# Cobalt-27/CompactFusion

Measured on AMD Instinct MI355X. Metric: residual_compressed_activation_exchange_throughput, higher is better.
Workload: dtype f16

## Files before the change

compactfusion_amd/csrc/cfx_absmean.hip:

```cpp
#include <hip/hip_runtime.h>
#include <hip/hip_ext.h>
#include <stdint.h>
#include <stdio.h>
#include <stdlib.h>
#include <string.h>
#include <algorithm>
#include "cfx.h"
#include "cfx_internal.h"
#include "cfx_device.h"
#include "cfx_host.h"

#define CFX_I_FLAG_LR_FACTORS_ONLY 0x100
#define CFX_I_FLAG_LR_ABS 0x200
extern "C" CFX_HIDDEN size_t cfx_i_lr_workspace_bytes_any(int N, int C, int rank, int batch);
extern "C" CFX_HIDDEN void cfx_i_lr_factor_offsets(int N, int C, int rank, size_t* offU16, size_t* offV16, size_t* per);

template <bool EMIT_BITS, int US, bool WT = false, int NW = WAVES, bool PUB = false, bool KEEP = false, bool TAG = false, class E = ElemF16>
__device__ __forceinline__ void absmean_stats_body(const cfx_comp_item& it, int N, int C, int R, int CB, int bx, int by,
                                                   u64* rowpart, u64 (*sm)[TILE_C], Probe probe = Probe(),
                                                   h16x8* xk = nullptr, h16x8* bk = nullptr, TagArena ta = TagArena()) {
#define SSTAMP(k) probe.at(k)
    const TileCoord t = tile_coord_at(bx, by, N, C, R);
    const int cb = bx;
    u64* colpart = rowpart + (size_t)N * CB;
    const h16* x = (const h16*)it.x;
    const h16* base = (const h16*)it.base;
    unsigned char* bitsout = (unsigned char*)it.packet;
    const int C8 = C >> 3;

    double col[8];
#pragma unroll
    for (int i = 0; i < 8; ++i) col[i] = 0.0;

    for (int r = t.r0 + t.w; r < t.r1; r += NW * US) {
        h16x8 xv[US], bv[US];
#pragma unroll
        for (int j = 0; j < US; ++j) {
            const int rr = r + NW * j;
            xv[j] = (h16x8)(h16)0;
            bv[j] = (h16x8)(h16)0;
            if (rr < t.r1 && t.act) {
                xv[j] = EMIT_BITS ? ld8nt(x + (size_t)rr * C + t.c) : ld8(x + (size_t)rr * C + t.c);
                if (base) bv[j] = ld8(base + (size_t)rr * C + t.c);
// ... 35 lines not shown
        }
        SSTAMP(9);
        u64 tot = 0;
#pragma unroll
        for (int j = 0; j < US; ++j) {
            const unsigned lo = wave_sum_u32_dpp((unsigned)(rs[j] & 0xffffffu));
            const unsigned hi = wave_sum_u32_dpp((unsigned)(rs[j] >> 24));
            const u64 tj = ((u64)hi << 24) + lo;
            if ((t.lane >> 4) == j) tot = tj;
        }
        SSTAMP(10);
        if ((t.lane & 15) == 0 && (t.lane >> 4) < US) {
            const int rr = r + NW * (t.lane >> 4);
            if (rr < t.r1) {
                if (TAG) put_tagged(ta.trow, rowpart, (size_t)cb * N + rr, tot, ta.tagbits);
                else if (WT) put_part(part32_of(rowpart, N, C, CB), rowpart, (size_t)cb * N + rr, tot);
                else rowpart[(size_t)cb * N + rr] = tot;
            }
        }
    }
#pragma unroll
    for (int i = 0; i < 8; ++i) sm[t.w][i * 64 + (t.lane ^ (i << 3))] = (u64)(col[i] * 16777216.0);
    SSTAMP(11);
    if (TAG && EMIT_BITS) asm volatile("s_waitcnt vmcnt(0)" ::: "memory");
    if (WT) lds_barrier(); else __syncthreads();
    SSTAMP(12);
    for (int k = threadIdx.x; k < TILE_C; k += NW * 64) {
        const int s = (k & 7) * 64 + ((k >> 3) ^ ((k & 7) << 3));
        const int cc = bx * TILE_C + k;
        if (cc < C) {
            u64 v = 0;
#pragma unroll
            for (int w = 0; w < NW; ++w) v += sm[w][s];
            if (TAG) put_tagged(ta.tcol, colpart, (size_t)by * C + cc, v, ta.tagbits);
            else if (WT) put_part(part32_of(rowpart, N, C, CB) + (size_t)N * CB, colpart, (size_t)by * C + cc, v);
            else colpart[(size_t)by * C + cc] = v;
        }
    }
#undef SSTAMP
}

template <bool EMIT_BITS, class E>
__global__ __launch_bounds__(NTHR) void k_absmean_stats(BatchC batch, int N, int C, int R, u64* ws, size_t ws_stride) {
    __shared__ u64 sm[WAVES][TILE_C];
    absmean_stats_body<EMIT_BITS, UNROLL_S, false, WAVES, false, false, false, E>(batch.it[blockIdx.z], N, C, R, gridDim.x, blockIdx.x, blockIdx.y, ws + (size_t)blockIdx.z * ws_stride, sm);
}

template <int NT>
__device__ __forceinline__ void absmean_finalize_body(const cfx_comp_item& it, int N, int C, int CB, int P, int per_byte, int eps_mode,
                                                      const u64* rowpart, int bx, u64* smem) {
    const u64* colpart = rowpart + (size_t)N * CB;
    h16* U = (h16*)((char*)it.packet + (size_t)N * (C / per_byte));
    h16* V = U + N;
    const int tid = threadIdx.x;
    if (bx == 0) {
        constexpr int KEEP = 3;
        u64 srow[KEEP];
        u64 acc = 0;
        int it_n = 0;
        for (int n = tid; n < N; n += NT, ++it_n) {
// ... 416 lines not shown
        for (int n0 = tid + 2 * NT; n0 - tid < N; n0 += 2 * NT) {
            const int n1 = n0 + NT;
            u64 s0, s1;
            row_sums2_wt(rowpart, row32, N, CB, min(n0, N - 1), min(n1, N - 1), (n1 & ~63) < N, s0, s1);
            if (n0 < N) PUT16(&U[n0], (h16)((float)mean16(s0, C) / den));
            if (n1 < N) PUT16(&U[n1], (h16)((float)mean16(s1, C) / den));
        }
        if (tid == 0) st_wt(tick + TICK_ALL, 0u);
    }
    if (last_col) {
        if (c < C) PUT16(&V[c], vmean);
        if (tid == 0) st_wt(tick + 1 + bx, 0u);
    }
#undef PUT16
    if (GATED) {
        asm volatile("s_waitcnt vmcnt(0)" ::: "memory");
        lds_barrier();
        if (tid == 0) gate_arrive_few(gate, (last_all ? 1u : 0u) + (last_col ? 1u : 0u));
    }
    STAMP(6);
#undef STAMP
}

__device__ __forceinline__ void absmean_tagged_jobs(const cfx_comp_item& it, int N, int C, int CB, int P, int bx, u64* rowpart, const TagArena& ta,
                                                    int per_byte, int eps_mode, u64 (*sm)[TILE_C], bool do_col, bool do_row, Probe probe,
                                                    unsigned* gate, unsigned* err, long long timeout) {
    constexpr int NT = FUSED_NT;
#define STAMP(k) probe.at(k)
    lds_barrier();
    const int tid = threadIdx.x;
    const u64* colpart = rowpart + (size_t)N * CB;
    h16* U = (h16*)((char*)it.packet + (size_t)N * (C / per_byte));
    h16* V = U + N;
    SpinClock clk;
    bool failed = false;
#define PUT16(ptr, val) st_wt((u16*)(ptr), hbits(val))
    if (do_col) {
        const int c = bx * TILE_C + tid, cc = min(c, C - 1);
        u64 a = 0;
        for (int p0 = 0; p0 < P && !failed; p0 += FUSED_CH) {
            u64 v[FUSED_CH];
            for (;;) {
#pragma unroll
                for (int j = 0; j < FUSED_CH; ++j) v[j] = ld_wt(&ta.tcol[(size_t)min(p0 + j, P - 1) * C + cc]);
                bool ok = true;
#pragma unroll
                for (int j = 0; j < FUSED_CH; ++j) ok = ok && tag_is(v[j], ta.tagbits);
                if (ok) break;
                __builtin_amdgcn_s_sleep(2);
                if (clk.expired(timeout)) { failed = true; break; }
            }
#pragma unroll
            for (int j = 0; j < FUSED_CH; ++j) {
                const u64 w = v[j] & TAG_SAT;
                if (p0 + j < P) a += (w == TAG_SAT && !failed) ? ld_wt(&colpart[(size_t)(p0 + j) * C + cc]) : w;
            }
        }
        STAMP(4);
        failed = __syncthreads_or(failed ? 1 : 0) != 0;
        if (!failed) {
            if (c < C) {
                const h16 vm = mean16(a, N);
                st_wt(&ta.tV[c], ta.tagbits | (u64)hbits(vm));
                PUT16(&V[c], vm);
            }
            asm volatile("s_waitcnt vmcnt(0)" ::: "memory");
            lds_barrier();
            if (tid == 0) gate_arrive_few(gate, 1u);
        }
        STAMP(5);
    }
    if (do_row && !failed) {
        u64* smem = &sm[1][0];
        auto row_sum = [&](int n) {
            const int nc = min(n, N - 1);
            u64 s_ = 0;
            for (int k0 = 0; k0 < CB && !failed; k0 += FUSED_RCH) {
                u64 q[FUSED_RCH];
                for (;;) {
#pragma unroll
                    for (int j = 0; j < FUSED_RCH; ++j) q[j] = ld_wt(&ta.trow[(size_t)min(k0 + j, CB - 1) * N + nc]);
                    bool ok = true;
#pragma unroll
                    for (int j = 0; j < FUSED_RCH; ++j) ok = ok && tag_is(q[j], ta.tagbits);
                    if (ok) break;
                    __builtin_amdgcn_s_sleep(2);
                    if (clk.expired(timeout)) { failed = true; break; }
                }
#pragma unroll
                for (int j = 0; j < FUSED_RCH; ++j) {
                    const u64 w = q[j] & TAG_SAT;
                    if (k0 + j < CB) s_ += (w == TAG_SAT && !failed) ? ld_wt(&rowpart[(size_t)(k0 + j) * N + nc]) : w;
                }
            }
// ... 77 lines not shown
        const int rr = t.r0 + t.w + NW * j;
        if (t.lane < 8 * US && rr < t.r1 && bx * TILE_C + seg * 64 < C)
            st16_wt(pk + (size_t)rr * (C >> 2) + bx * (TILE_C >> 2) + seg * 16, *(const u32x4*)(smw + j * 128 + seg * 16));
    }
    asm volatile("s_waitcnt vmcnt(0)" ::: "memory");
    lds_barrier();
    if (threadIdx.x == 0) {
        st_wt(&ta.tdone[(size_t)bx * ((N + R - 1) / R) + by], ta.tagbits);
        gate_arrive(gate2, 1u, expect2);
    }
    if (upd) {
#pragma unroll
        for (int j = 0; j < US; ++j) {
            const int rr = t.r0 + t.w + NW * j;
            const h16 tk = hfrom((u16)__builtin_amdgcn_readlane((int)ul, j));
            if (rr < t.r1 && t.act) {
                const h16x8 recv = int2_recv(codes[j], ch8 * tk);
                st8nt(nb + (size_t)rr * C + t.c, ef ? (el_state<E>(has_base, bk[j], recv)) : xk[j]);
            }
        }
    }
}

template <bool EMIT_BITS, int US, bool GATED = false, bool KEEP = false, class E = ElemF16>
__device__ __forceinline__ void absmean_fused_body(const cfx_comp_item& it, int N, int C, int R, int CB, int P, int bx, int by,
                                                   u64* rowpart, unsigned* tick, int per_byte, int eps_mode, u64 (*sm)[TILE_C], int dbg,
                                                   Probe probe, unsigned* gate = nullptr, unsigned gate_expect = 0, int flags = 0,
                                                   unsigned* gate2 = nullptr, unsigned expect2 = 0, unsigned* err = nullptr, long long timeout = 0,
                                                   TagArena ta = TagArena()) {
#define STAMP(k) probe.at(k)
    STAMP(0);
#ifdef CFX_DEV_PROBES
    if (dbg == 3) return;
    if (dbg == 4) {
        const TileCoord t = tile_coord_at(bx, by, N, C, R);
        h16x8 acc = (h16x8)(h16)0;
        for (int r = t.r0 + t.w; r < t.r1; r += FUSED_NW * US) {
            h16x8 xv[US], bv[US];
#pragma unroll
            for (int j = 0; j < US; ++j) {
                const int rr = min(r + FUSED_NW * j, t.r1 - 1);
                xv[j] = ld8nt((const h16*)it.x + (size_t)rr * C + min(t.c, C - 8));
                bv[j] = ld8((const h16*)it.base + (size_t)rr * C + min(t.c, C - 8));
            }
#pragma unroll
            for (int j = 0; j < US; ++j) acc += xv[j] - bv[j];
        }
        if (acc[0] == (h16)12345.0f) ((h16*)it.packet)[threadIdx.x] = acc[1];
        return;
    }
#endif
    h16x8 xk[KEEP ? US : 1], bk[KEEP ? US : 1];
    absmean_stats_body<EMIT_BITS, US, true, FUSED_NW, GATED, KEEP, GATED, E>(it, N, C, R, CB, bx, by, rowpart, sm, probe, xk, bk, ta);
    STAMP(1);
    if constexpr (GATED) {
        const bool v_wg = by == P - 1;
        const bool u_wg = P >= 2 ? (by == P - 2 && bx == CB - 1) : (bx == CB - 1);
        probe.copy(2, 1); probe.copy(3, 1); probe.set(7, (v_wg ? 1 : 0) | (u_wg ? 2 : 0));
        if (v_wg || u_wg) {
            u32x4* park = (u32x4*)&sm[FUSED_NW][0];
            if constexpr (KEEP) {
                park[threadIdx.x] = __builtin_bit_cast(u32x4, xk[US - 1]);
                park[FUSED_NT + threadIdx.x] = __builtin_bit_cast(u32x4, bk[US - 1]);
            }
            absmean_tagged_jobs(it, N, C, CB, P, bx, rowpart, ta, per_byte, eps_mode, sm, v_wg, u_wg, probe, gate, err, timeout);
            if constexpr (KEEP) {
                xk[US - 1] = __builtin_bit_cast(h16x8, park[threadIdx.x]);
                bk[US - 1] = __builtin_bit_cast(h16x8, park[FUSED_NT + threadIdx.x]);
            }
        }
    } else {
    asm volatile("s_waitcnt vmcnt(0)" ::: "memory");
    __syncthreads();
    STAMP(2);
#ifdef CFX_DEV_PROBES
    if (dbg == 1) return;
#endif
    unsigned* flag = (unsigned*)&sm[0][0];
    if (threadIdx.x == 0) flag[0] = __hip_atomic_fetch_add(tick + 1 + bx, 1u, __ATOMIC_RELAXED, __HIP_MEMORY_SCOPE_AGENT);
    if (threadIdx.x == 64) (void)__hip_atomic_fetch_add(tick + TICK_ALL, 1u, __ATOMIC_RELAXED, __HIP_MEMORY_SCOPE_AGENT);
    lds_barrier();
    const bool last_col = flag[0] == (unsigned)(P - 1);
    const bool u_wg = bx == 0 && by == 0;
    STAMP(3);
    probe.set(7, (last_col ? 1 : 0) | (u_wg ? 2 : 0));
#ifdef CFX_DEV_PROBES
    if (dbg == 2) {
        if (last_col && threadIdx.x == 0) st_wt(tick + 1 + bx, 0u);
// ... 30 lines not shown
    int n_st;
    int dq_R, dq_rb;
    int per_byte, eps_mode;
    int dbg;
    u64* ws;
    size_t ws_stride;
    unsigned* tick;
    Probe probe;
    int n_g, g_R, g_rb, n_gt;
    unsigned* gate;
    unsigned gate_expect;
    unsigned* gate_err;
    long long timeout;
    u64* tarena; size_t tarena_stride; unsigned tag;
    signed char src[CFX_MAX_BATCH];
    unsigned* xgate;
    unsigned xexpect;
    int remote;
    P2PInline p2p;
};
#ifndef GATE_WPE
#define GATE_WPE 4
#endif
template <bool EMIT_BITS, int US, bool GATED, bool ST, class E>
__global__ __launch_bounds__(FUSED_NT, GATE_WPE) __attribute__((amdgpu_num_vgpr(52))) void k_absmean_compress(BatchC batch, BatchD ride, BatchD gated, FusedArgs a) {
    __shared__ u64 sm[FUSED_NW][TILE_C];
    int b = blockIdx.x;
    if (b < a.n_st) {
        const int per = a.CB * a.P;
        const int z = b / per, rem = b - z * per;
        const int by = rem / a.CB;
        absmean_fused_body<EMIT_BITS, US, GATED, false, E>(batch.it[z], a.N, a.C, a.R, a.CB, a.P, rem - by * a.CB, by, a.ws + (size_t)z * a.ws_stride,
                                                 a.tick + z * TICK_WORDS, a.per_byte, a.eps_mode, sm, a.dbg,
                                                 a.probe.of(b), a.gate, a.gate_expect, 0, nullptr, 0u, a.gate_err, a.timeout,
                                                 tag_arena_of(a.tarena, a.tarena_stride, z, a.N, a.C, a.CB, a.P, a.tag));
        if constexpr (GATED) {
            if (b == 0 && a.p2p.own) p2p_exchange_inline(a.gate, a.gate_expect, 1, a.p2p, a.xgate, a.xexpect, a.gate_err);
        }
        return;
    }
    if constexpr (EMIT_BITS) {
        b -= a.n_st;
        if constexpr (GATED) {
            if (b < a.n_g) {
                const int per = a.CB * a.g_rb;
                for (int t = b; t < a.n_gt; t += a.n_g) {
                    const int item = t / per, rem = t - item * per;
                    const int ty = rem / a.CB;
                    const int sz = a.src[item];
                    const TagArena ta = tag_arena_of(a.tarena, a.tarena_stride, sz >= 0 ? sz : 0, a.N, a.C, a.CB, a.P, a.tag);
                    binary_dequant_gated_body<FUSED_NW, GATE_KR, 0, ST, E>(gated.it[item], a.N, a.C, a.g_R, rem - ty * a.CB, ty, a.xgate ? a.xgate : a.gate,
                                                                a.xgate ? a.xexpect : a.gate_expect, a.gate_err, a.timeout,
                                                                nullptr,
                                                                a.probe.of(blockIdx.x), a.remote != 0 && sz < 0,
                                                                ONEBIT_D_TAGGED && sz >= 0, ta, (u16*)&sm[0][0]);
                }
                return;
            }
            b -= a.n_g;
        }
        const int per = a.CB * a.dq_rb;
        const int item = b / per, rem = b - item * per;
        const int ty = rem / a.CB;
        binary_dequant_body<FUSED_NW, UNROLL, E>(ride.it[item], a.N, a.C, a.dq_R, rem - ty * a.CB, ty);
    }
}

#ifndef PIPE_US
#define PIPE_US 2
#endif
#define PIPE_MAX_DQ CFX_PIPE_MAX_DQ
struct BatchDX { cfx_decomp_item it[PIPE_MAX_DQ]; };
struct PipeArgs {
    int N, C, CB;
    int n_fin, fin_bpi, fin_P;
    int n_st, st_R, st_P;
    int dq_R, dq_rb;
    const u64* ws_fin;
    u64* ws_st;
    size_t ws_stride;
};
template <bool STEADY>
__global__ __launch_bounds__(NTHR) __attribute__((amdgpu_waves_per_eu(8, 8))) void k_binary_pipe(BatchDX dq, BatchC fin, BatchC st, PipeArgs a) {
    __shared__ u64 sm[WAVES][TILE_C];
    int b = blockIdx.x;
    if (b < a.n_fin) {
        const int item = b / a.fin_bpi;
        absmean_finalize_body<NTHR>(fin.it[item], a.N, a.C, a.CB, a.fin_P, 8, 0, a.ws_fin + (size_t)item * a.ws_stride, b - item * a.fin_bpi, &sm[0][0]);
// ... 198 lines not shown
    }
}

#ifndef INT2_D_TAGGED
#define INT2_D_TAGGED 1
#endif
struct Int2LayerArgs {
    int N, C, CB, R, P, n_st;
    int g_R, g_rb, n_g;
    int flags;
    u64* ws;
    size_t ws_stride;
    unsigned* tick;
    unsigned* gate1; unsigned expect1;
    unsigned* gate2; unsigned expect2;
    unsigned* err;
    long long timeout;
    u64* tarena; size_t tarena_stride; unsigned tag;
    signed char src[CFX_MAX_BATCH];
    unsigned* xgate; unsigned xexpect;
    int remote;
    P2PInline p2p;
};
template <int US, class E>
__global__ __launch_bounds__(FUSED_NT, 4) void k_int2_compress_gated(BatchC batch, BatchD gated, Int2LayerArgs a) {
    __shared__ u64 sm[(GATE_LDS_ROWS > FUSED_NW + 4 ? GATE_LDS_ROWS : FUSED_NW + 4) + 1][TILE_C];
    int b = blockIdx.x;
    if (b < a.n_st) {
        const int per = a.CB * a.P;
        const int z = b / per, rem = b - z * per;
        const int by = rem / a.CB;
        absmean_fused_body<false, US, true, true, E>(batch.it[z], a.N, a.C, a.R, a.CB, a.P, rem - by * a.CB, by, a.ws + (size_t)z * a.ws_stride,
                                                  a.tick + z * TICK_WORDS, 4, 1, sm, 0, Probe(), a.gate1, a.expect1, a.flags, a.gate2, a.expect2, a.err, a.timeout,
                                                  tag_arena_of(a.tarena, a.tarena_stride, z, a.N, a.C, a.CB, a.P, a.tag));
        if (b == 0 && a.p2p.own) p2p_exchange_inline(a.gate2 + 1 * GATE_LINE, a.expect2, 1, a.p2p, a.xgate, a.xexpect, a.err);
        return;
    }
    b -= a.n_st;
    const int per = a.CB * a.g_rb;
    const int item = b / per, rem = b - item * per;
    const int ty = rem / a.CB;
    const int sz = a.src[item];
    const TagArena ta = tag_arena_of(a.tarena, a.tarena_stride, sz >= 0 ? sz : 0, a.N, a.C, a.CB, a.P, a.tag);
    int2_dequant_gated_body<FUSED_NW, GATE_KR2, GATE_KL, E>(gated.it[item], a.N, a.C, a.g_R, rem - ty * a.CB, ty, a.gate2, a.expect2, a.err, a.timeout,
                                                        (u32x4*)&sm[0][0], a.xgate, a.xexpect, a.remote != 0 && sz < 0, INT2_D_TAGGED && sz >= 0, ta, a.R,
                                                        (u16*)&sm[GATE_LDS_ROWS][0]);
}


#define LAUNCH_EL(bf16, ...) do { \
        if (bf16) { using EL = ElemBF16; LAUNCH(__VA_ARGS__); } \
        else { using EL = ElemF16; LAUNCH(__VA_ARGS__); } \
    } while (0)

static bool gated_one_launch(cfx_ctx* ctx, int codec, int C, int CB) {
    return (codec == CFX_CODEC_BINARY || codec == CFX_CODEC_INT2) && ctx->fused && CB <= TICK_MAX_CB && C % 128 == 0 && !ctx->dev_probe && ctx->gated_on;
}

static unsigned abs_arena_for(cfx_ctx* ctx, unsigned ring, void* stream, size_t need_bytes, u64** arena) {
    hipStream_t s = (hipStream_t)stream;
    if (!ctx->mml_arena_owned[ring] || ctx->mml_arena_owner[ring] != stream) {
        if (ctx->mml_arena_owned[ring]) (void)hipDeviceSynchronize();
        ctx->mml_arena_owner[ring] = stream;
        ctx->mml_arena_owned[ring] = true;
    }
    if (ctx->abs_arena_bytes[ring] < need_bytes) {
        if (ctx->abs_arena[ring]) (void)hipFree(ctx->abs_arena[ring]);
        ctx->abs_arena[ring] = nullptr;
        ctx->abs_arena_bytes[ring] = 0;
// ... 90 lines not shown
        ctx->gate_expect[3 * slot + 1] += (unsigned)a.n_st;
        a.expect1 = ctx->gate_expect[3 * slot]; a.expect2 = ctx->gate_expect[3 * slot + 1];
        a.err = ctx->gate_err;
        a.timeout = ctx->gate_timeout;
        a.tarena_stride = tag_arena_words(N, C, CB, P);
        a.tag = abs_arena_for(ctx, slot / TICK_RING, stream, a.tarena_stride * batch * sizeof(u64), &a.tarena);
        if (!a.tag) return fail(ctx, CFX_ERR_LAUNCH, "2-bit layer launch: cannot allocate the partials' arena");
        for (int g_ = 0; g_ < n_gated; ++g_) {
            a.src[g_] = -1;
            for (int i = 0; i < batch; ++i)
                if (gd.it[g_].packet == items[i].packet) a.src[g_] = (signed char)i;
        }
        if (xg) {
            a.xgate = a.gate1 + 2 * GATE_BLOCK;
            a.xexpect = ++ctx->gate_expect[3 * slot + 2];
            a.remote = xg->remote;
            fill_p2p(ctx, xg, a.p2p);
            xg->taken = 1;
            xg->p_gate = a.gate2 + 1 * GATE_LINE;
            xg->p_expect = a.expect2;
            xg->f_gate = a.xgate; xg->f_expect = a.xexpect;
        }
        const dim3 g(a.n_st + a.n_g);
        LAUNCH_EL(bf16, ctx, KID_ABSMEAN_COMPRESS_GATED, s, (k_int2_compress_gated<4, EL>), g, dim3(FUSED_NT), 0, s, b, gd, a);
        return check_launch(ctx, "2-bit layer launch");
    }
    const bool ef_gated = one_launch && codec == CFX_CODEC_BINARY && upd && !(flags & CFX_FLAG_NO_EF) && n_gated + batch <= CFX_MAX_BATCH;
    const bool one_launch_1bit = one_launch && codec == CFX_CODEC_BINARY && (!upd || ef_gated);
    int n_gated_k = n_gated;
    if (ef_gated) {
        for (int i = n_gated - 1; i >= 0; --i) gd.it[i + batch] = gd.it[i];
        for (int i = 0; i < batch; ++i) { gd.it[i].packet = items[i].packet; gd.it[i].base = items[i].base; gd.it[i].recon = items[i].new_base; }
        n_gated_k = n_gated + batch;
    }
    if (fused) {
        FusedArgs a;
        memset(&a, 0, sizeof(a));
        a.N = N; a.C = C; a.CB = CB; a.R = R; a.P = P;
        a.n_st = CB * P * batch;
        a.dq_R = FUSED_NW * UNROLL;
        a.dq_rb = (N + a.dq_R - 1) / a.dq_R;
        a.per_byte = per_byte; a.eps_mode = codec == CFX_CODEC_INT2 ? 1 : 0;
        a.ws = ws; a.ws_stride = wstride; a.tick = tick;
        a.dbg = ctx->dev_probe;
        a.probe = cfx_i_probe(ctx);
        if (one_launch_1bit) {
            a.g_rb = (N + FUSED_NW * GATE_KR - 1) / (FUSED_NW * GATE_KR);
// ... 3 lines not shown
            ctx->gate_expect[3 * slot] += (unsigned)batch * (unsigned)(CB + 1);
            a.gate_expect = ctx->gate_expect[3 * slot];
            a.tarena_stride = tag_arena_words(N, C, CB, P);
            a.tag = abs_arena_for(ctx, slot / TICK_RING, stream, a.tarena_stride * batch * sizeof(u64), &a.tarena);
            if (!a.tag) return fail(ctx, CFX_ERR_LAUNCH, "1-bit layer launch: cannot allocate the partials' arena");
            for (int g_ = 0; g_ < n_gated_k; ++g_) {
                a.src[g_] = -1;
                for (int i = 0; i < batch; ++i)
                    if (gd.it[g_].packet == items[i].packet) a.src[g_] = (signed char)i;
            }
            if (xg) {
                a.xgate = a.gate + GATE_BLOCK;
                a.xexpect = ++ctx->gate_expect[3 * slot + 1];
                a.remote = xg->remote;
                fill_p2p(ctx, xg, a.p2p);
                xg->taken = 1;
                xg->p_gate = a.gate; xg->p_expect = a.gate_expect;
                xg->f_gate = a.xgate; xg->f_expect = a.xexpect;
            }
        }
        a.gate_err = ctx->gate_err;
        a.timeout = ctx->gate_timeout;
        const dim3 g(a.n_st + a.n_g + CB * a.dq_rb * n_ride);
#ifdef CFX_DEV_PROBES
        if (one_launch_1bit && ctx->dev_buf && R % 32 == 0) {
            LAUNCH_EL(bf16, ctx, KID_ABSMEAN_COMPRESS_GATED, s, (k_absmean_compress<true, 4, true, true, EL>), g, dim3(FUSED_NT), 0, s, b, rd, gd, a);
        } else
#endif
        if (one_launch_1bit) {
            LAUNCH_EL(bf16, ctx, KID_ABSMEAN_COMPRESS_GATED, s, (k_absmean_compress<true, 4, true, false, EL>), g, dim3(FUSED_NT), 0, s, b, rd, gd, a);
        } else if (codec == CFX_CODEC_BINARY) {
            if (R % 32 == 0) LAUNCH_EL(bf16, ctx, KID_ABSMEAN_COMPRESS_BITS, s, (k_absmean_compress<true, 4, false, false, EL>), g, dim3(FUSED_NT), 0, s, b, rd, gd, a);
            else LAUNCH_EL(bf16, ctx, KID_ABSMEAN_COMPRESS_BITS, s, (k_absmean_compress<true, 2, false, false, EL>), g, dim3(FUSED_NT), 0, s, b, rd, gd, a);
        } else {
            if (R % 32 == 0) LAUNCH_EL(bf16, ctx, KID_ABSMEAN_COMPRESS, s, (k_absmean_compress<false, 4, false, false, EL>), g, dim3(FUSED_NT), 0, s, b, rd, gd, a);
            else LAUNCH_EL(bf16, ctx, KID_ABSMEAN_COMPRESS, s, (k_absmean_compress<false, 2, false, false, EL>), g, dim3(FUSED_NT), 0, s, b, rd, gd, a);
        }
    } else {
        if (codec == CFX_CODEC_BINARY) LAUNCH_EL(bf16, ctx, KID_ABSMEAN_STATS_BITS, s, (k_absmean_stats<true, EL>), grid, dim3(NTHR), 0, s, b, N, C, R, ws, wstride);
        else LAUNCH_EL(bf16, ctx, KID_ABSMEAN_STATS, s, (k_absmean_stats<false, EL>), grid, dim3(NTHR), 0, s, b, N, C, R, ws, wstride);
        LAUNCH(ctx, KID_ABSMEAN_FINALIZE, s, k_absmean_finalize, dim3(1 + (C + 255) / 256, batch), dim3(1024), 0, s, b, N, C, CB, P, per_byte,
                           codec == CFX_CODEC_INT2 ? 1 : 0, (const u64*)ws, wstride);
        if (n_ride) {
            const int Rr = auto_rows(ctx, N, C, n_ride, false);
            LAUNCH_EL(bf16, ctx, KID_BINARY_DEQUANT, s, (k_binary_dequant<UNROLL, EL>), dim3(CB, (N + Rr - 1) / Rr, n_ride), dim3(NTHR), 0, s, rd, N, C, Rr, (unsigned*)nullptr, 0u);
        }
    }
    if (codec == CFX_CODEC_INT2) {
        LAUNCH_EL(bf16, ctx, KID_INT2_QUANT, s, (k_int2_quant<EL>), gridq, dim3(NTHR), 0, s, b, N, C, Rq, flags);
    } else if (upd && !one_launch_1bit) {
        if (flags & CFX_FLAG_NO_EF) {
            for (int i = 0; i < batch; ++i)
// ... 178 lines not shown
```

compactfusion_amd/csrc/cfx_api.hip:

```cpp
#include <hip/hip_runtime.h>
#include <hip/hip_ext.h>
#include <stdint.h>
#include <stdio.h>
#include <stdlib.h>
#include <string.h>
#include <algorithm>
#include "cfx.h"
#include "cfx_internal.h"
#include "cfx_device.h"
#define CFX_API_TU
#include "cfx_host.h"

__global__ __launch_bounds__(256) void k_residual2_delta(const h16* __restrict__ x, const h16* base, const h16* dbase, h16* dd, size_t n8) {
    const size_t i = (size_t)blockIdx.x * 256 + threadIdx.x;
    if (i >= n8) return;
    const h16x8 d = ld8nt(x + i * 8) - ld8(base + i * 8);
    st8(dd + i * 8, d - ld8(dbase + i * 8));
}
__global__ __launch_bounds__(256) void k_residual2_update(const h16* base, const h16* dbase, const h16* __restrict__ recv, h16* nb, h16* ndb,
                                                          float decay, size_t n8) {
    const size_t i = (size_t)blockIdx.x * 256 + threadIdx.x;
    if (i >= n8) return;
    const h16x8 b = ld8(base + i * 8), d = ld8(dbase + i * 8), r = ld8nt(recv + i * 8);
    const h16x8 pred = b + d;
// ... 142 lines not shown
    c->device = device;
    c->rows_per_tile = 0;
    c->prof = nullptr;
    c->prof_cap = c->prof_n = 0;
    c->prof_stride = 1;
    memset(c->prof_seen, 0, sizeof(c->prof_seen));
    c->prof_mask = 0;
    c->tick = nullptr;
    memset(c->tick_next, 0, sizeof(c->tick_next));
    c->n_ring_streams = 0;
    c->n_cu_cache = 0;
    c->cu_cache_next = 0;
    c->ring_clock = 0;
    memset(c->ring_used, 0, sizeof(c->ring_used));
    c->dev_buf = nullptr;
    c->gate = nullptr;
    c->gate_err = nullptr;
    c->gate_timeout = 500000000LL;
    c->fused = 1;
    c->stats_rows = 0;
    c->gated_on = 1;
    c->lr_chain = c->lr_decode = 0;
    c->dev_probe = 0;
    c->allow_shared_queues = 0;
    c->ipc_kind = 0;
    c->ipc_want = 2;
    c->err[0] = 0;
    return c;
}

int cfx_prepare(cfx_ctx* ctx) {
    if (!ctx) return CFX_ERR_NULL;
    if (ctx->tick) return CFX_OK;
    int cur = -1;
    (void)hipGetDevice(&cur);
    if (cur != ctx->device && hipSetDevice(ctx->device) != hipSuccess) return fail(ctx, CFX_ERR_LAUNCH, "prepare: hipSetDevice failed");
    static_assert(3 * TICK_RING * CFX_RING_STREAMS == sizeof(((cfx_ctx*)0)->gate_expect) / sizeof(unsigned), "gate_expect has three entries per ring slot");
    const size_t tick_words = (size_t)CFX_RING_STREAMS * TICK_RING * CFX_MAX_BATCH * TICK_WORDS;
    const size_t gate_words = (size_t)(CFX_RING_STREAMS * TICK_RING + 1) * GATE_STRIDE;
    const size_t colgate_words = (size_t)CFX_RING_STREAMS * MML_MAX_TILES;
    const size_t bytes = (tick_words + gate_words + colgate_words) * sizeof(unsigned);
    void* p = nullptr;
    int rc = CFX_OK;
    if (hipMalloc(&p, bytes) != hipSuccess || hipMemset(p, 0, bytes) != hipSuccess || hipDeviceSynchronize() != hipSuccess) {
        (void)hipGetLastError();
        if (p) (void)hipFree(p);
// ... 10 lines not shown
    }
    if (cur >= 0 && cur != ctx->device) (void)hipSetDevice(cur);
    return rc;
}

#ifdef CFX_DEV_PROBES
int cfx_dev_stamps(cfx_ctx* ctx, void* buf) {
    if (!ctx) return CFX_ERR_NULL;
    ctx->dev_buf = buf;
    return CFX_OK;
}

int cfx_dev_set_launch_tags(cfx_ctx* ctx, unsigned abs_seq, unsigned mml_seq) {
    if (!ctx) return CFX_ERR_NULL;
    if (!ctx->tick && cfx_prepare(ctx) != CFX_OK) return CFX_ERR_LAUNCH;
    (void)hipDeviceSynchronize();
    ctx->abs_seq = abs_seq;
    ctx->mml_seq = mml_seq;
    return CFX_OK;
}

int cfx_dev_set_probe(cfx_ctx* ctx, int mode) {
    if (!ctx) return CFX_ERR_NULL;
    if (mode < 0 || mode > 4) return fail(ctx, CFX_ERR_BATCH, "dev probe must be 0..4");
    ctx->dev_probe = mode;
    return CFX_OK;
}
#endif

int cfx_set_fused_finalize(cfx_ctx* ctx, int on) {
    if (!ctx) return CFX_ERR_NULL;
    ctx->fused = on != 0;
    return CFX_OK;
}

int cfx_set_stats_rows(cfx_ctx* ctx, int rows) {
    if (!ctx) return CFX_ERR_NULL;
    if (rows < 0 || rows > 4096) return fail(ctx, CFX_ERR_BATCH, "stats rows must be 0 (automatic) .. 4096");
    ctx->stats_rows = rows;
    return CFX_OK;
}

int cfx_set_gated_launch(cfx_ctx* ctx, int on) {
    if (!ctx) return CFX_ERR_NULL;
    ctx->gated_on = on != 0;
    return CFX_OK;
}

int cfx_set_lr_chain(cfx_ctx* ctx, int chain) {
    if (!ctx) return CFX_ERR_NULL;
    if (chain < 0 || chain > 2) return fail(ctx, CFX_ERR_BATCH, "lr chain must be 0 (automatic), 1 (no single launch) or 2 (C-space chain)");
    ctx->lr_chain = chain;
    return CFX_OK;
}

int cfx_set_lr_decode(cfx_ctx* ctx, int mode) {
    if (!ctx) return CFX_ERR_NULL;
    if (mode < 0 || mode > 2) return fail(ctx, CFX_ERR_BATCH, "lr decode must be 0 (automatic), 1 (VALU) or 2 (MFMA)");
    ctx->lr_decode = mode;
    return CFX_OK;
}

int cfx_set_allow_shared_queues(cfx_ctx* ctx, int on) {
    if (!ctx) return CFX_ERR_NULL;
    ctx->allow_shared_queues = on != 0;
    return CFX_OK;
}

// ... 429 lines not shown
```

compactfusion_amd/csrc/cfx_device.h:

```cpp
#ifndef CFX_DEVICE_H
#define CFX_DEVICE_H
#include <hip/hip_runtime.h>
#include <stdint.h>
#include "cfx.h"
#include "cfx_internal.h"

typedef _Float16 h16;
typedef h16 h16x8 __attribute__((ext_vector_type(8)));
typedef unsigned short u16;
typedef u16 u16x8 __attribute__((ext_vector_type(8)));
typedef unsigned long long u64;
typedef unsigned u32x4 __attribute__((ext_vector_type(4)));
typedef float f32x2 __attribute__((ext_vector_type(2)));
typedef h16 h16x2 __attribute__((ext_vector_type(2)));
typedef __bf16 bf16x2 __attribute__((ext_vector_type(2)));

#define TILE_C 512
#define WAVES 4
#define NTHR (WAVES * 64)
#define UNROLL 2
#define UNROLL_S 4

struct BatchC { cfx_comp_item it[CFX_MAX_BATCH]; };
struct BatchD { cfx_decomp_item it[CFX_MAX_BATCH]; };
// ... 201 lines not shown
    t.lane = threadIdx.x & 63;
    t.w = __builtin_amdgcn_readfirstlane(threadIdx.x >> 6);
    t.c = bx * TILE_C + t.lane * 8;
    t.act = t.c < C;
    t.r0 = by * R;
    t.r1 = min(N, t.r0 + R);
    return t;
}
__device__ __forceinline__ TileCoord tile_coord(int N, int C, int R) { return tile_coord_at(blockIdx.x, blockIdx.y, N, C, R); }

#define MML_MAX_TILES 2048
#define TICK_WORDS 64
#define TICK_ALL 48
#define TICK_MAX_CB 46
#define TICK_RING 256

#define FUSED_NW 8
#define FUSED_NT (FUSED_NW * 64)
#ifndef FUSED_CH
#define FUSED_CH 18

#endif
#define FUSED_RCH 6

#ifndef GATE_KR
#define GATE_KR 14
#endif
#ifndef GATE_KR2
#define GATE_KR2 17

#endif
#ifndef GATE_KL
#define GATE_KL 6
#endif
#define GATE_LDS_ROWS ((GATE_KL * FUSED_NT * 16 + TILE_C * 8 - 1) / (TILE_C * 8))
#ifndef GATE_LOCAL_SLEEP
#define GATE_LOCAL_SLEEP 1

#endif
#define GATE_LINE 16
#define GATE_BLOCK (25 * GATE_LINE)
#define GATE_STRIDE (3 * GATE_BLOCK)
__device__ __forceinline__ void gate_arrive_few(unsigned* gate, unsigned inc) {
    (void)__hip_atomic_fetch_add(gate, inc, __ATOMIC_RELAXED, __HIP_MEMORY_SCOPE_AGENT);
}
__device__ __forceinline__ void gate_arrive(unsigned* gate, unsigned inc, unsigned expect) {
// ... 116 lines not shown
```

compactfusion_amd/csrc/cfx_internal.h:

```cpp
#ifndef CFX_INTERNAL_H
#define CFX_INTERNAL_H
#include <hip/hip_runtime.h>
#include <hip/hip_ext.h>
#include <stdint.h>
#include <stdio.h>
#include "cfx.h"
#ifdef CFX_DEV_PROBES
#include "cfx_dev.h"
#endif

enum {
    KID_ABSMEAN_STATS_BITS = 1, KID_ABSMEAN_STATS = 2, KID_ABSMEAN_FINALIZE = 3, KID_BINARY_DEQUANT = 4,
    KID_INT2_QUANT = 5, KID_INT2_DEQUANT = 6, KID_MINMAX_STATS = 7, KID_MINMAX_FINALIZE = 8,
    KID_INT8_QUANT = 9, KID_INT8_DEQUANT = 10, KID_INT4_QUANT = 11, KID_INT4_DEQUANT = 12,
    KID_TOPK_COMPRESS = 13, KID_TOPK_DECOMPRESS = 14, KID_COPY_PROBE = 15, KID_BINARY_EF = 16,
    KID_LR_PREP = 17, KID_LR_AQ = 18, KID_LR_ATY = 19, KID_LR_CHOL = 20, KID_LR_APPLY = 21, KID_LR_DECODE = 22,
    KID_BINARY_PIPE = 23, KID_BINARY_PIPE_EDGE = 24, KID_RES2_DELTA = 25, KID_RES2_UPDATE = 26,
    KID_ABSMEAN_COMPRESS_BITS = 27, KID_ABSMEAN_COMPRESS = 28, KID_MINMAX_COMPRESS = 29, KID_ATTN_MERGE = 30,
    KID_ABSMEAN_COMPRESS_GATED = 31, KID_MAX = 32,
    KID_LR_CHAIN = KID_LR_PREP
};
static const char* const kid_names[KID_MAX] = {
    "", "k_absmean_stats<bits>", "k_absmean_stats", "k_absmean_finalize", "k_binary_dequant", "k_int2_quant", "k_int2_dequant",
    "k_minmax_stats", "k_minmax_finalize", "k_int8_quant", "k_int8_dequant", "k_int4_quant", "k_int4_dequant",
// ... 40 lines not shown
    void* ring_stream[CFX_RING_STREAMS];
    int n_ring_streams;
    unsigned long long ring_used[CFX_RING_STREAMS], ring_clock;
    void* cu_cache_stream[8];
    int cu_cache_n[8], n_cu_cache;
    unsigned cu_cache_next;
    unsigned* gate;
    unsigned gate_expect[3 * 256 * CFX_RING_STREAMS];
    unsigned* colgate;
    unsigned mml_seq;
    unsigned long long* mml_arena[CFX_RING_STREAMS];
    size_t mml_arena_bytes[CFX_RING_STREAMS];
    bool mml_arena_owned[CFX_RING_STREAMS];
    void* mml_arena_owner[CFX_RING_STREAMS];
    unsigned long long* abs_arena[CFX_RING_STREAMS];
    size_t abs_arena_bytes[CFX_RING_STREAMS];
    unsigned abs_seq;
    unsigned* gate_err;
    long long gate_timeout;
    int fused;
    void* dev_buf;
    int stats_rows;
    int gated_on;
    int lr_chain, lr_decode;
    int dev_probe;
    int allow_shared_queues;
    int ipc_want;
    int ipc_kind;
    void* lrs_stream[8];
    char* lrs_arena[8];
    size_t lrs_bytes[8];
    unsigned long long lrs_key[8];
    int lrs_n;
    unsigned lrs_next;
    void* lrs_last_stream;
    hipEvent_t lrs_ev;
    char err[256];
};

static inline Probe cfx_i_probe(const cfx_ctx* ctx) {
#ifdef CFX_DEV_PROBES
    return Probe((unsigned long long*)ctx->dev_buf);
#else
    (void)ctx;
    return Probe();
#endif
// ... 144 lines not shown
```

Before: 2118.

## Restructure the 1-bit scale chain into a one-round U job with landed counter

Adds a chain variant of the gated absmean compress kernel. The row-mean (U) job now does its tagged polling in a single round over two row blocks per thread, and a per-item 'landed' atomic counter replaces the per-block wait on bit stores before the barrier. The tagged U/V publish stores are dropped when the consumer is not tagged-reading. This is meant to shorten the cross-workgroup dependency chain and cut redundant global stores in the fused one-launch layer. The cost is an extra counter wait and a reset per round, plus more template instantiations. gated_on=2 keeps the old path.

```diff
diff --git a/compactfusion_amd/csrc/cfx_absmean.hip b/compactfusion_amd/csrc/cfx_absmean.hip
--- a/compactfusion_amd/csrc/cfx_absmean.hip
+++ b/compactfusion_amd/csrc/cfx_absmean.hip
@@ -15,10 +15,11 @@
 extern "C" CFX_HIDDEN size_t cfx_i_lr_workspace_bytes_any(int N, int C, int rank, int batch);
 extern "C" CFX_HIDDEN void cfx_i_lr_factor_offsets(int N, int C, int rank, size_t* offU16, size_t* offV16, size_t* per);
 
-template <bool EMIT_BITS, int US, bool WT = false, int NW = WAVES, bool PUB = false, bool KEEP = false, bool TAG = false, class E = ElemF16>
+template <bool EMIT_BITS, int US, bool WT = false, int NW = WAVES, bool PUB = false, bool KEEP = false, bool TAG = false, class E = ElemF16,
+          int CHAIN = 0>
 __device__ __forceinline__ void absmean_stats_body(const cfx_comp_item& it, int N, int C, int R, int CB, int bx, int by,
                                                    u64* rowpart, u64 (*sm)[TILE_C], Probe probe = Probe(),
-                                                   h16x8* xk = nullptr, h16x8* bk = nullptr, TagArena ta = TagArena()) {
+                                                   h16x8* xk = nullptr, h16x8* bk = nullptr, TagArena ta = TagArena(), unsigned* landed = nullptr) {
 #define SSTAMP(k) probe.at(k)
     const TileCoord t = tile_coord_at(bx, by, N, C, R);
     const int cb = bx;
@@ -100,7 +101,7 @@
 #pragma unroll
     for (int i = 0; i < 8; ++i) sm[t.w][i * 64 + (t.lane ^ (i << 3))] = (u64)(col[i] * 16777216.0);
     SSTAMP(11);
-    if (TAG && EMIT_BITS) asm volatile("s_waitcnt vmcnt(0)" ::: "memory");
+    if (TAG && EMIT_BITS && !(CHAIN & CHAIN_LANDED)) asm volatile("s_waitcnt vmcnt(0)" ::: "memory");
     if (WT) lds_barrier(); else __syncthreads();
     SSTAMP(12);
     for (int k = threadIdx.x; k < TILE_C; k += NW * 64) {
@@ -114,6 +115,11 @@
             else if (WT) put_part(part32_of(rowpart, N, C, CB) + (size_t)N * CB, colpart, (size_t)by * C + cc, v);
             else colpart[(size_t)by * C + cc] = v;
         }
+    }
+    if constexpr (TAG && EMIT_BITS && (CHAIN & CHAIN_LANDED) != 0) {
+        asm volatile("s_waitcnt vmcnt(0)" ::: "memory");
+        lds_barrier();
+        if (threadIdx.x == 0) (void)__hip_atomic_fetch_add(landed, 1u, __ATOMIC_RELAXED, __HIP_MEMORY_SCOPE_AGENT);
     }
 #undef SSTAMP
 }
@@ -576,9 +582,118 @@
 #undef STAMP
 }
 
+template <int CHAIN>
+__device__ __forceinline__ bool absmean_u_job_round(h16* U, int N, int C, int CB, int P, const u64* rowpart, const TagArena& ta, int eps_mode,
+                                                    u64* smem, Probe probe, unsigned* gate, unsigned* landed, long long timeout, SpinClock& clk) {
+    constexpr int NT = FUSED_NT, RB = FUSED_RB;
+    const int tid = threadIdx.x;
+    bool failed = false;
+    bool look = (CHAIN & CHAIN_LANDED) != 0 && tid == 0;
+    unsigned seen = 0;
+    auto row_sums = [&](int nb, u64 (&s_)[RB]) {
+#pragma unroll
+        for (int i = 0; i < RB; ++i) s_[i] = 0;
+        for (int k0 = 0; k0 < CB && !failed; k0 += FUSED_RCH) {
+            u64 q[RB][FUSED_RCH];
+            bool ok[RB];
+#pragma unroll
+            for (int i = 0; i < RB; ++i) {
+                ok[i] = nb + i * NT >= N;
+#pragma unroll
+                for (int j = 0; j < FUSED_RCH; ++j) q[i][j] = 0;
+            }
+            for (;;) {
+#pragma unroll
+                for (int i = 0; i < RB; ++i)
+                    if (!ok[i]) {
+#pragma unroll
+                        for (int j = 0; j < FUSED_RCH; ++j)
+                            q[i][j] = ld_wt((const u64*)((const char*)(ta.trow + (size_t)min(k0 + j, CB - 1) * N) + (unsigned)(nb + i * NT) * 8u));
+                    }
+                if (look) { seen = ld_wt(landed); look = false; }
+                bool all = true;
+#pragma unroll
+                for (int i = 0; i < RB; ++i)
+                    if (!ok[i]) {
+                        bool o = true;
+#pragma unroll
+                        for (int j = 0; j < FUSED_RCH; ++j) o = o && tag_is(q[i][j], ta.tagbits);
+                        ok[i] = o;
+                        all = all && o;
+                    }
+                if (all) break;
+                __builtin_amdgcn_s_sleep(2);
+                if (clk.expired(timeout)) { failed = true; break; }
+            }
+#pragma unroll
+            for (int i = 0; i < RB; ++i) {
+#pragma unroll
+                for (int j = 0; j < FUSED_RCH; ++j) {
+                    const u64 w = q[i][j] & TAG_SAT;
+                    if (k0 + j < CB) s_[i] += (w == TAG_SAT && !failed) ? ld_wt(&rowpart[(size_t)(k0 + j) * N + nb + i * NT]) : w;
+                }
+            }
+        }
+    };
+    h16 hk[RB];
+#pragma unroll
+    for (int i = 0; i < RB; ++i) hk[i] = (h16)0;
+    u64 acc = 0;
+    for (int nb = tid, b = 0; nb - tid < N; nb += RB * NT, ++b) {
+        u64 s_[RB];
+        row_sums(nb, s_);
+#pragma unroll
+        for (int i = 0; i < RB; ++i) {
+            const h16 h = mean16(s_[i], C);
+            if (b == 0) hk[i] = h;
+            if (nb + i * NT < N) acc += habs_units(hbits(h));
+        }
+    }
+    probe.at(13);
+    const u64 wtot = wave_sum_u64(acc);
+    if ((tid & 63) == 0) smem[tid >> 6] = wtot;
+    failed = __syncthreads_or(failed ? 1 : 0) != 0;
+    probe.at(15);
+    if (failed) return true;
+    u64 tot = 0;
+#pragma unroll
+    for (int w = 0; w < NT / 64; ++w) tot += smem[w];
+    const h16 mu = mean16(tot, N);
+    const float den = eps_mode ? (float)(h16)((float)mu + 1e-6f) : (float)mu;
+    for (int nb = tid, b = 0; nb < N; nb += RB * NT, ++b) {
+        u64 s_[RB];
+        if (b > 0) row_sums(nb, s_);
+#pragma unroll
+        for (int i = 0; i < RB; ++i) {
+            const int n = nb + i * NT;
+            if (n < N) {
+                const h16 h = b == 0 ? hk[i] : mean16(s_[i], C);
+                const h16 un = (h16)((float)h / den);
+                if (!(CHAIN & CHAIN_NOTAG)) st_wt(&ta.tU[n], ta.tagbits | (u64)hbits(un));
+                st_wt((u16*)&U[n], hbits(un));
+            }
+        }
+    }
+    asm volatile("s_waitcnt vmcnt(0)" ::: "memory");
+    if ((CHAIN & CHAIN_LANDED) != 0 && tid == 0) {
+        while (seen != (unsigned)(CB * P)) {
+            seen = ld_wt(landed);
+            if (seen == (unsigned)(CB * P)) break;
+            __builtin_amdgcn_s_sleep(1);
+            if (clk.expired(timeout)) { failed = true; break; }
+        }
+        if (!failed) st_wt(landed, 0u);
+    }
+    lds_barrier();
+    if (tid == 0 && !failed) gate_arrive_few(gate, 1u);
+    probe.at(6);
+    return failed;
+}
+
+template <int CHAIN = 0>
 __device__ __forceinline__ void absmean_tagged_jobs(const cfx_comp_item& it, int N, int C, int CB, int P, int bx, u64* rowpart, const TagArena& ta,
                                                     int per_byte, int eps_mode, u64 (*sm)[TILE_C], bool do_col, bool do_row, Probe probe,
-                                                    unsigned* gate, unsigned* err, long long timeout) {
+                                                    unsigned* gate, unsigned* err, long long timeout, unsigned* landed = nullptr) {
     constexpr int NT = FUSED_NT;
 #define STAMP(k) probe.at(k)
     lds_barrier();
@@ -615,7 +730,7 @@
         if (!failed) {
             if (c < C) {
                 const h16 vm = mean16(a, N);
-                st_wt(&ta.tV[c], ta.tagbits | (u64)hbits(vm));
+                if (!(CHAIN & CHAIN_NOTAG)) st_wt(&ta.tV[c], ta.tagbits | (u64)hbits(vm));
                 PUT16(&V[c], vm);
             }
             asm volatile("s_waitcnt vmcnt(0)" ::: "memory");
@@ -624,6 +739,10 @@
         }
         STAMP(5);
     }
+    if constexpr ((CHAIN & CHAIN_ROUND) != 0) {
+        if (do_row && !failed)
+            failed = absmean_u_job_round<CHAIN>(U, N, C, CB, P, rowpart, ta, eps_mode, &sm[1][0], probe, gate, landed, timeout, clk);
+    } else
     if (do_row && !failed) {
         u64* smem = &sm[1][0];
         auto row_sum = [&](int n) {
@@ -747,7 +866,7 @@
     }
 }
 
-template <bool EMIT_BITS, int US, bool GATED = false, bool KEEP = false, class E = ElemF16>
+template <bool EMIT_BITS, int US, bool GATED = false, bool KEEP = false, class E = ElemF16, int CHAIN = 0>
 __device__ __forceinline__ void absmean_fused_body(const cfx_comp_item& it, int N, int C, int R, int CB, int P, int bx, int by,
                                                    u64* rowpart, unsigned* tick, int per_byte, int eps_mode, u64 (*sm)[TILE_C], int dbg,
                                                    Probe probe, unsigned* gate = nullptr, unsigned gate_expect = 0, int flags = 0,
@@ -776,7 +895,7 @@
     }
 #endif
     h16x8 xk[KEEP ? US : 1], bk[KEEP ? US : 1];
-    absmean_stats_body<EMIT_BITS, US, true, FUSED_NW, GATED, KEEP, GATED, E>(it, N, C, R, CB, bx, by, rowpart, sm, probe, xk, bk, ta);
+    absmean_stats_body<EMIT_BITS, US, true, FUSED_NW, GATED, KEEP, GATED, E, CHAIN>(it, N, C, R, CB, bx, by, rowpart, sm, probe, xk, bk, ta, tick + TICK_ALL);
     STAMP(1);
     if constexpr (GATED) {
         const bool v_wg = by == P - 1;
@@ -788,7 +907,7 @@
                 park[threadIdx.x] = __builtin_bit_cast(u32x4, xk[US - 1]);
                 park[FUSED_NT + threadIdx.x] = __builtin_bit_cast(u32x4, bk[US - 1]);
             }
-            absmean_tagged_jobs(it, N, C, CB, P, bx, rowpart, ta, per_byte, eps_mode, sm, v_wg, u_wg, probe, gate, err, timeout);
+            absmean_tagged_jobs<CHAIN>(it, N, C, CB, P, bx, rowpart, ta, per_byte, eps_mode, sm, v_wg, u_wg, probe, gate, err, timeout, tick + TICK_ALL);
             if constexpr (KEEP) {
                 xk[US - 1] = __builtin_bit_cast(h16x8, park[threadIdx.x]);
                 bk[US - 1] = __builtin_bit_cast(h16x8, park[FUSED_NT + threadIdx.x]);
@@ -865,15 +984,14 @@
 #ifndef GATE_WPE
 #define GATE_WPE 4
 #endif
-template <bool EMIT_BITS, int US, bool GATED, bool ST, class E>
-__global__ __launch_bounds__(FUSED_NT, GATE_WPE) __attribute__((amdgpu_num_vgpr(52))) void k_absmean_compress(BatchC batch, BatchD ride, BatchD gated, FusedArgs a) {
-    __shared__ u64 sm[FUSED_NW][TILE_C];
+template <bool EMIT_BITS, int US, bool GATED, bool ST, class E, int CHAIN>
+__device__ __forceinline__ void absmean_compress_launch(const BatchC& batch, const BatchD& ride, const BatchD& gated, const FusedArgs& a, u64 (*sm)[TILE_C]) {
     int b = blockIdx.x;
     if (b < a.n_st) {
         const int per = a.CB * a.P;
         const int z = b / per, rem = b - z * per;
         const int by = rem / a.CB;
-        absmean_fused_body<EMIT_BITS, US, GATED, false, E>(batch.it[z], a.N, a.C, a.R, a.CB, a.P, rem - by * a.CB, by, a.ws + (size_t)z * a.ws_stride,
+        absmean_fused_body<EMIT_BITS, US, GATED, false, E, CHAIN>(batch.it[z], a.N, a.C, a.R, a.CB, a.P, rem - by * a.CB, by, a.ws + (size_t)z * a.ws_stride,
                                                  a.tick + z * TICK_WORDS, a.per_byte, a.eps_mode, sm, a.dbg,
                                                  a.probe.of(b), a.gate, a.gate_expect, 0, nullptr, 0u, a.gate_err, a.timeout,
                                                  tag_arena_of(a.tarena, a.tarena_stride, z, a.N, a.C, a.CB, a.P, a.tag));
@@ -896,7 +1014,7 @@
                                                                 a.xgate ? a.xexpect : a.gate_expect, a.gate_err, a.timeout,
                                                                 nullptr,
                                                                 a.probe.of(blockIdx.x), a.remote != 0 && sz < 0,
-                                                                ONEBIT_D_TAGGED && sz >= 0, ta, (u16*)&sm[0][0]);
+                                                                ONEBIT_D_TAGGED && !(CHAIN & CHAIN_NOTAG) && sz >= 0, ta, (u16*)&sm[0][0]);
                 }
                 return;
             }
@@ -907,6 +1025,17 @@
         const int ty = rem / a.CB;
         binary_dequant_body<FUSED_NW, UNROLL, E>(ride.it[item], a.N, a.C, a.dq_R, rem - ty * a.CB, ty);
     }
+}
+template <bool EMIT_BITS, int US, bool GATED, bool ST, class E>
+__global__ __launch_bounds__(FUSED_NT, GATE_WPE) __attribute__((amdgpu_num_vgpr(52))) void k_absmean_compress(BatchC batch, BatchD ride, BatchD gated, FusedArgs a) {
+    __shared__ u64 sm[FUSED_NW][TILE_C];
+    absmean_compress_launch<EMIT_BITS, US, GATED, ST, E, 0>(batch, ride, gated, a, sm);
+}
+template <bool EMIT_BITS, int US, bool GATED, bool ST, class E, int CHAIN>
+__global__ __launch_bounds__(FUSED_NT, GATE_WPE) __attribute__((amdgpu_num_vgpr(52))) void k_absmean_compress(BatchC batch, BatchD ride, BatchD gated, FusedArgs a) {
+    static_assert(EMIT_BITS && GATED && CHAIN != 0, "chain forms exist for the 1-bit layer launch only");
+    __shared__ u64 sm[FUSED_NW][TILE_C];
+    absmean_compress_launch<EMIT_BITS, US, GATED, ST, E, CHAIN>(batch, ride, gated, a, sm);
 }
 
 #ifndef PIPE_US
@@ -1151,15 +1280,15 @@
     int remote;
     P2PInline p2p;
 };
-template <int US, class E>
-__global__ __launch_bounds__(FUSED_NT, 4) void k_int2_compress_gated(BatchC batch, BatchD gated, Int2LayerArgs a) {
-    __shared__ u64 sm[(GATE_LDS_ROWS > FUSED_NW + 4 ? GATE_LDS_ROWS : FUSED_NW + 4) + 1][TILE_C];
+#define INT2_LAYER_LDS_ROWS ((GATE_LDS_ROWS > FUSED_NW + 4 ? GATE_LDS_ROWS : FUSED_NW + 4) + 1)
+template <int US, class E, int CHAIN>
+__device__ __forceinline__ void int2_layer_launch(const BatchC& batch, const BatchD& gated, const Int2LayerArgs& a, u64 (*sm)[TILE_C]) {
     int b = blockIdx.x;
     if (b < a.n_st) {
         const int per = a.CB * a.P;
         const int z = b / per, rem = b - z * per;
         const int by = rem / a.CB;
-        absmean_fused_body<false, US, true, true, E>(batch.it[z], a.N, a.C, a.R, a.CB, a.P, rem - by * a.CB, by, a.ws + (size_t)z * a.ws_stride,
+        absmean_fused_body<false, US, true, true, E, CHAIN>(batch.it[z], a.N, a.C, a.R, a.CB, a.P, rem - by * a.CB, by, a.ws + (size_t)z * a.ws_stride,
                                                   a.tick + z * TICK_WORDS, 4, 1, sm, 0, Probe(), a.gate1, a.expect1, a.flags, a.gate2, a.expect2, a.err, a.timeout,
                                                   tag_arena_of(a.tarena, a.tarena_stride, z, a.N, a.C, a.CB, a.P, a.tag));
         if (b == 0 && a.p2p.own) p2p_exchange_inline(a.gate2 + 1 * GATE_LINE, a.expect2, 1, a.p2p, a.xgate, a.xexpect, a.err);
@@ -1174,6 +1303,17 @@
     int2_dequant_gated_body<FUSED_NW, GATE_KR2, GATE_KL, E>(gated.it[item], a.N, a.C, a.g_R, rem - ty * a.CB, ty, a.gate2, a.expect2, a.err, a.timeout,
                                                         (u32x4*)&sm[0][0], a.xgate, a.xexpect, a.remote != 0 && sz < 0, INT2_D_TAGGED && sz >= 0, ta, a.R,
                                                         (u16*)&sm[GATE_LDS_ROWS][0]);
+}
+template <int US, class E>
+__global__ __launch_bounds__(FUSED_NT, 4) void k_int2_compress_gated(BatchC batch, BatchD gated, Int2LayerArgs a) {
+    __shared__ u64 sm[INT2_LAYER_LDS_ROWS][TILE_C];
+    int2_layer_launch<US, E, 0>(batch, gated, a, sm);
+}
+template <int US, class E, int CHAIN>
+__global__ __launch_bounds__(FUSED_NT, 4) void k_int2_compress_gated(BatchC batch, BatchD gated, Int2LayerArgs a) {
+    static_assert(CHAIN == CHAIN_ROUND, "the 2-bit layer launch takes the one-round U job only");
+    __shared__ u64 sm[INT2_LAYER_LDS_ROWS][TILE_C];
+    int2_layer_launch<US, E, CHAIN>(batch, gated, a, sm);
 }
 
 
@@ -1310,7 +1450,8 @@
             xg->f_gate = a.xgate; xg->f_expect = a.xexpect;
         }
         const dim3 g(a.n_st + a.n_g);
-        LAUNCH_EL(bf16, ctx, KID_ABSMEAN_COMPRESS_GATED, s, (k_int2_compress_gated<4, EL>), g, dim3(FUSED_NT), 0, s, b, gd, a);
+        if (ctx->gated_on == 2) LAUNCH_EL(bf16, ctx, KID_ABSMEAN_COMPRESS_GATED, s, (k_int2_compress_gated<4, EL>), g, dim3(FUSED_NT), 0, s, b, gd, a);
+        else LAUNCH_EL(bf16, ctx, KID_ABSMEAN_COMPRESS_GATED, s, (k_int2_compress_gated<4, EL, CHAIN_ROUND>), g, dim3(FUSED_NT), 0, s, b, gd, a);
         return check_launch(ctx, "2-bit layer launch");
     }
     const bool ef_gated = one_launch && codec == CFX_CODEC_BINARY && upd && !(flags & CFX_FLAG_NO_EF) && n_gated + batch <= CFX_MAX_BATCH;
@@ -1360,12 +1501,19 @@
         a.gate_err = ctx->gate_err;
         a.timeout = ctx->gate_timeout;
         const dim3 g(a.n_st + a.n_g + CB * a.dq_rb * n_ride);
+        int chain = ctx->gated_on == 2 ? 0 : CHAIN_1BIT;
 #ifdef CFX_DEV_PROBES
+        if (chain) chain = ctx->dev_chain;
         if (one_launch_1bit && ctx->dev_buf && R % 32 == 0) {
-            LAUNCH_EL(bf16, ctx, KID_ABSMEAN_COMPRESS_GATED, s, (k_absmean_compress<true, 4, true, true, EL>), g, dim3(FUSED_NT), 0, s, b, rd, gd, a);
+            if (chain == CHAIN_1BIT) LAUNCH_EL(bf16, ctx, KID_ABSMEAN_COMPRESS_GATED, s, (k_absmean_compress<true, 4, true, true, EL, CHAIN_1BIT>), g, dim3(FUSED_NT), 0, s, b, rd, gd, a);
+            else if (chain == (CHAIN_ROUND | CHAIN_LANDED)) LAUNCH_EL(bf16, ctx, KID_ABSMEAN_COMPRESS_GATED, s, (k_absmean_compress<true, 4, true, true, EL, CHAIN_ROUND | CHAIN_LANDED>), g, dim3(FUSED_NT), 0, s, b, rd, gd, a);
+            else if (chain == CHAIN_ROUND) LAUNCH_EL(bf16, ctx, KID_ABSMEAN_COMPRESS_GATED, s, (k_absmean_compress<true, 4, true, true, EL, CHAIN_ROUND>), g, dim3(FUSED_NT), 0, s, b, rd, gd, a);
+            else LAUNCH_EL(bf16, ctx, KID_ABSMEAN_COMPRESS_GATED, s, (k_absmean_compress<true, 4, true, true, EL>), g, dim3(FUSED_NT), 0, s, b, rd, gd, a);
         } else
 #endif
-        if (one_launch_1bit) {
+        if (one_launch_1bit && chain) {
+            LAUNCH_EL(bf16, ctx, KID_ABSMEAN_COMPRESS_GATED, s, (k_absmean_compress<true, 4, true, false, EL, CHAIN_1BIT>), g, dim3(FUSED_NT), 0, s, b, rd, gd, a);
+        } else if (one_launch_1bit) {
             LAUNCH_EL(bf16, ctx, KID_ABSMEAN_COMPRESS_GATED, s, (k_absmean_compress<true, 4, true, false, EL>), g, dim3(FUSED_NT), 0, s, b, rd, gd, a);
         } else if (codec == CFX_CODEC_BINARY) {
             if (R % 32 == 0) LAUNCH_EL(bf16, ctx, KID_ABSMEAN_COMPRESS_BITS, s, (k_absmean_compress<true, 4, false, false, EL>), g, dim3(FUSED_NT), 0, s, b, rd, gd, a);
diff --git a/compactfusion_amd/csrc/cfx_api.hip b/compactfusion_amd/csrc/cfx_api.hip
--- a/compactfusion_amd/csrc/cfx_api.hip
+++ b/compactfusion_amd/csrc/cfx_api.hip
@@ -188,6 +188,7 @@
     c->gated_on = 1;
     c->lr_chain = c->lr_decode = 0;
     c->dev_probe = 0;
+    c->dev_chain = 7;
     c->allow_shared_queues = 0;
     c->ipc_kind = 0;
     c->ipc_want = 2;
@@ -244,6 +245,13 @@
 
 int cfx_dev_set_probe(cfx_ctx* ctx, int mode) {
     if (!ctx) return CFX_ERR_NULL;
+    if (mode & 0x100) {
+        const int chain = mode & 0xff;
+        if (mode >> 9 || (chain != CHAIN_ROUND && chain != (CHAIN_ROUND | CHAIN_LANDED) && chain != CHAIN_1BIT))
+            return fail(ctx, CFX_ERR_BATCH, "dev probe: the chain pieces are 0x101, 0x103 or 0x107");
+        ctx->dev_chain = chain;
+        return CFX_OK;
+    }
     if (mode < 0 || mode > 4) return fail(ctx, CFX_ERR_BATCH, "dev probe must be 0..4");
     ctx->dev_probe = mode;
     return CFX_OK;
@@ -265,7 +273,8 @@
 
 int cfx_set_gated_launch(cfx_ctx* ctx, int on) {
     if (!ctx) return CFX_ERR_NULL;
-    ctx->gated_on = on != 0;
+    if (on < 0 || on > 2) return fail(ctx, CFX_ERR_BATCH, "gated launch must be 0 (off), 1 (the one-launch forms) or 2 (one launch, the 1-bit scale chain as it was)");
+    ctx->gated_on = on;
     return CFX_OK;
 }
 
diff --git a/compactfusion_amd/csrc/cfx_device.h b/compactfusion_amd/csrc/cfx_device.h
--- a/compactfusion_amd/csrc/cfx_device.h
+++ b/compactfusion_amd/csrc/cfx_device.h
@@ -247,6 +247,11 @@
 
 #endif
 #define FUSED_RCH 6
+#define CHAIN_ROUND 1
+#define CHAIN_LANDED 2
+#define CHAIN_NOTAG 4
+#define CHAIN_1BIT (CHAIN_ROUND | CHAIN_LANDED | CHAIN_NOTAG)
+#define FUSED_RB 2
 
 #ifndef GATE_KR
 #define GATE_KR 14
diff --git a/compactfusion_amd/csrc/cfx_internal.h b/compactfusion_amd/csrc/cfx_internal.h
--- a/compactfusion_amd/csrc/cfx_internal.h
+++ b/compactfusion_amd/csrc/cfx_internal.h
@@ -86,6 +86,7 @@
     void* dev_buf;
     int stats_rows;
     int gated_on;
+    int dev_chain;
     int lr_chain, lr_decode;
     int dev_probe;
     int allow_shared_queues;
```

After: 2151, median of 6. No clear change (+1.6%).
